# chenc10/distributed_TensorFlow_models

Hardware: AMD Instinct MI355X
Metric: images/sec (whole node) ResNet-50 224×224 bf16 at 1/2/4/8 MI355X (higher is better)
Workload: dtype bf16; 1 GPU; model=resnet_v1_50, global_batch=256, per_gpu_batch=256, image_size=224, parallelism=dp1, device=cuda, grad_allreduce_dtype=fp32, deterministic=True, optimizer=momentum-sgd+wd

## Files before the change

### csrc/kernels/batchnorm.hip

```cpp
#include "common.h"

namespace dtm {

template <int V>
struct Vec;
template <>
struct Vec<8> {
  uint4 u;
  __device__ __forceinline__ void load(const bf16_t* p) { u = *(const uint4*)p; }
  __device__ __forceinline__ void store(bf16_t* p) const { *(uint4*)p = u; }
  __device__ __forceinline__ float get(int e) const {
    uint32_t w = e < 2 ? u.x : e < 4 ? u.y : e < 6 ? u.z : u.w;
    return (e & 1) ? hi_bf(w) : lo_bf(w);
  }
  __device__ __forceinline__ void unpack(float* f) const {
    f[0] = lo_bf(u.x); f[1] = hi_bf(u.x); f[2] = lo_bf(u.y); f[3] = hi_bf(u.y);
    f[4] = lo_bf(u.z); f[5] = hi_bf(u.z); f[6] = lo_bf(u.w); f[7] = hi_bf(u.w);
  }
  __device__ __forceinline__ void pack(const float* f) {
    u = make_uint4(pack2bf(f[0], f[1]), pack2bf(f[2], f[3]), pack2bf(f[4], f[5]), pack2bf(f[6], f[7]));
  }
};
template <>
struct Vec<1> {
// ... 249 lines not shown
}


__global__ __launch_bounds__(256) void bn_stats_fast(const bf16_t* __restrict__ x, float* __restrict__ stats, int M,
                                                     int C, int rpb) {
  __shared__ float red[2][256][8];
  const int cols = C >> 3, t = threadIdx.x, RP = 256 / cols, c0 = (t % cols) * 8, lr0 = t / cols;
  const int r0 = blockIdx.x * rpb, r1 = min(M, r0 + rpb);
  float s[8], q[8];
#pragma unroll
  for (int e = 0; e < 8; ++e) s[e] = q[e] = 0.f;
  for (int r = lr0 < RP ? r0 + lr0 : r1; r < r1; r += RP * FU) {
    uint4 v[FU];
#pragma unroll
    for (int u = 0; u < FU; ++u) {
      int rr = r + u * RP;
      v[u] = rr < r1 ? *(const uint4*)(x + (size_t)rr * C + c0) : make_uint4(0, 0, 0, 0);
    }
#pragma unroll
    for (int u = 0; u < FU; ++u) {
      float f[8]; unpack8(v[u], f);
#pragma unroll
      for (int e = 0; e < 8; ++e) { s[e] += f[e]; q[e] += f[e] * f[e]; }
    }
  }
  col_reduce8(red, s, q, stats + (size_t)blockIdx.x * 2 * C, stats + (size_t)blockIdx.x * 2 * C + C, cols, c0);
}

typedef unsigned int v4u_bn_t __attribute__((ext_vector_type(4)));
template <bool NT>
__device__ __forceinline__ uint4 ld16_bn(const bf16_t* p) {
  if (NT) {
    v4u_bn_t v = __builtin_nontemporal_load((const v4u_bn_t*)p);
    return make_uint4(v.x, v.y, v.z, v.w);
  }
  return *(const uint4*)p;
}

template <bool NT>
__global__ __launch_bounds__(256) void bn_apply_fast(const bf16_t* __restrict__ x, const float* __restrict__ ss,
                                                     const bf16_t* __restrict__ res, const float* __restrict__ rss,
                                                     bf16_t* __restrict__ y, uint8_t* __restrict__ mask, int M, int C,
                                                     int res_mode, int relu, int rpb, int ldy) {
  const int cols = C >> 3, t = threadIdx.x, RP = 256 / cols, c0 = (t % cols) * 8, lr0 = t / cols;
  float sc[8], sh[8], rsc[8], rsh[8];
#pragma unroll
  for (int e = 0; e < 8; ++e) {
    sc[e] = ss[c0 + e]; sh[e] = ss[C + c0 + e];
    rsc[e] = res_mode == 2 ? rss[c0 + e] : 1.f;
    rsh[e] = res_mode == 2 ? rss[C + c0 + e] : 0.f;
  }
  const int r0 = blockIdx.x * rpb, r1 = min(M, r0 + rpb);
  for (int r = lr0 < RP ? r0 + lr0 : r1; r < r1; r += RP * FU) {
    uint4 v[FU], w[FU];
#pragma unroll
    for (int u = 0; u < FU; ++u) {
      int rr = r + u * RP;
      bool ok = rr < r1;
      v[u] = ok ? ld16_bn<NT>(x + (size_t)rr * C + c0) : make_uint4(0, 0, 0, 0);
      if (res_mode) w[u] = ok ? ld16_bn<NT>(res + (size_t)rr * C + c0) : make_uint4(0, 0, 0, 0);
    }
#pragma unroll
    for (int u = 0; u < FU; ++u) {
      int rr = r + u * RP;
      if (rr >= r1) break;
      float f[8]; unpack8(v[u], f);
#pragma unroll
      for (int e = 0; e < 8; ++e) f[e] = fmaf(f[e], sc[e], sh[e]);
      if (res_mode) {
        float g[8]; unpack8(w[u], g);
#pragma unroll
        for (int e = 0; e < 8; ++e) f[e] += fmaf(g[e], rsc[e], rsh[e]);
      }
      if (relu) {
        uint32_t bits = 0;
#pragma unroll
        for (int e = 0; e < 8; ++e) {
          bits |= (f[e] > 0.f ? 1u : 0u) << e;
          f[e] = fmaxf(f[e], 0.f);
        }
        if (mask) mask[((size_t)rr * C + c0) >> 3] = (uint8_t)bits;
      }
      *(uint4*)(y + (size_t)rr * ldy + c0) = pack8(f);
    }
  }
}

__global__ __launch_bounds__(256) void bn_apply_res_strided(const bf16_t* __restrict__ x, const float* __restrict__ ss,
                                                            const bf16_t* __restrict__ res, bf16_t* __restrict__ y,
                                                            uint8_t* __restrict__ mask,
                                                            uint32_t M, int C, int relu, FastDiv fd_cols, FastDiv fd_Wo,
                                                            FastDiv fd_Ho, int Ho, int Wo, int Hi, int Wi, int s) {
  const uint32_t cols = C >> 3, total = M * cols;
  for (uint32_t i = blockIdx.x * 256u + threadIdx.x; i < total; i += gridDim.x * 256u) {
    const uint32_t r = fdiv(i, fd_cols), c0 = (i - r * cols) * 8;
    const uint32_t t = fdiv(r, fd_Wo), w = r - t * Wo;
    const uint32_t n = fdiv(t, fd_Ho), h = t - n * Ho;
    const size_t rr = ((size_t)n * Hi + (size_t)h * s) * Wi + (size_t)w * s;
    float f[8], g[8];
    unpack8(*(const uint4*)(x + (size_t)r * C + c0), f);
    unpack8(*(const uint4*)(res + rr * C + c0), g);
    uint32_t bits = 0;
#pragma unroll
    for (int e = 0; e < 8; ++e) {
      f[e] = fmaf(f[e], ss[c0 + e], ss[C + c0 + e]) + g[e];
      bits |= (f[e] > 0.f ? 1u : 0u) << e;
      if (relu) f[e] = fmaxf(f[e], 0.f);
    }
    if (relu && mask) mask[((size_t)r * C + c0) >> 3] = (uint8_t)bits;
    *(uint4*)(y + (size_t)r * C + c0) = pack8(f);
  }
}

__global__ __launch_bounds__(256) void bn_bwd_reduce_fast(const bf16_t* __restrict__ dy, const bf16_t* __restrict__ x,
                                                          const bf16_t* __restrict__ ym, const float* __restrict__ ss,
                                                          float* __restrict__ sums, int M, int C, int mask_mode, int rpb) {
  __shared__ float red[2][256][8];
  const int cols = C >> 3, t = threadIdx.x, RP = 256 / cols, c0 = (t % cols) * 8, lr0 = t / cols;
  float sc[8], sh[8], mu[8], rs[8];
#pragma unroll
  for (int e = 0; e < 8; ++e) {
    sc[e] = ss[c0 + e]; sh[e] = ss[C + c0 + e]; mu[e] = ss[2 * C + c0 + e]; rs[e] = ss[3 * C + c0 + e];
  }
  const int r0 = blockIdx.x * rpb, r1 = min(M, r0 + rpb);
  float s[8], q[8];
#pragma unroll
  for (int e = 0; e < 8; ++e) s[e] = q[e] = 0.f;
  for (int r = lr0 < RP ? r0 + lr0 : r1; r < r1; r += RP * FU) {
    uint4 a[FU], b[FU], m[FU];
#pragma unroll
    for (int u = 0; u < FU; ++u) {
      int rr = r + u * RP;
      bool ok = rr < r1;
      size_t o = (size_t)rr * C + c0;
      a[u] = ok ? *(const uint4*)(dy + o) : make_uint4(0, 0, 0, 0);
      b[u] = ok ? *(const uint4*)(x + o) : make_uint4(0, 0, 0, 0);
      if (mask_mode == 1) m[u] = ok ? *(const uint4*)(ym + o) : make_uint4(0, 0, 0, 0);
    }
#pragma unroll
    for (int u = 0; u < FU; ++u) {
      float g[8], xv[8];
      unpack8(a[u], g); unpack8(b[u], xv);
      if (mask_mode == 1) {
        float mv[8]; unpack8(m[u], mv);
#pragma unroll
        for (int e = 0; e < 8; ++e) g[e] = mv[e] > 0.f ? g[e] : 0.f;
      } else if (mask_mode == 2) {
#pragma unroll
        for (int e = 0; e < 8; ++e) g[e] = fmaf(xv[e], sc[e], sh[e]) > 0.f ? g[e] : 0.f;
      }
#pragma unroll
      for (int e = 0; e < 8; ++e) { s[e] += g[e]; q[e] += g[e] * (xv[e] - mu[e]) * rs[e]; }
    }
  }
  col_reduce8(red, s, q, sums + (size_t)blockIdx.x * 2 * C, sums + (size_t)blockIdx.x * 2 * C + C, cols, c0);
}

__global__ __launch_bounds__(256) void bn_bwd_apply_fast(const bf16_t* __restrict__ dy, const bf16_t* __restrict__ x,
                                                         const bf16_t* __restrict__ ym, const float* __restrict__ ss,
                                                         const float* __restrict__ sums, bf16_t* __restrict__ dx,
                                                         bf16_t* __restrict__ gout, int M, int C, int mask_mode,
                                                         int training, int rpb) {
  const int cols = C >> 3, t = threadIdx.x, RP = 256 / cols, c0 = (t % cols) * 8, lr0 = t / cols;
  const float invM = 1.f / (float)M;
  float sc[8], sh[8], mu[8], rs[8], A[8], Bq[8];
#pragma unroll
// ... 222 lines not shown
  long blocks = (n8 + 255) / 256;
  if (blocks > 8192) blocks = 8192;
  hipLaunchKernelGGL(bn_stats_bwd_kernel, dim3((unsigned)blocks), dim3(256), 0, (hipStream_t)stream, (const bf16_t*)y,
                     dstats, (const bf16_t*)g, (bf16_t*)dy, n8, C / 8);
  return 0;
}

DTM_API void dtm_bn_stats(const void* x, float* stats, long M, int C, void* stream) {
  if (fast_ok(M, C)) {
    int blocks, rpb; fast_grid(M, C, &blocks, &rpb);
    float* ws = dtm_ws_get_stream((size_t)blocks * 2 * C, (hipStream_t)stream);
    hipLaunchKernelGGL(bn_stats_fast, dim3(blocks), dim3(256), 0, (hipStream_t)stream, (const bf16_t*)x, ws, (int)M, C, rpb);
    dtm_reduce_rows(ws, blocks, 2 * C, 2 * C, stats, (hipStream_t)stream);
    return;
  }
  long rpb = rows_per_block_for(M, C);
  int blocks = (int)((M + rpb - 1) / rpb);
  if (C % 8 == 0)
    hipLaunchKernelGGL(bn_stats_kernel<8>, dim3(blocks), dim3(256), 0, (hipStream_t)stream, (const bf16_t*)x, stats, M, C, rpb);
  else
    hipLaunchKernelGGL(bn_stats_kernel<1>, dim3(blocks), dim3(256), 0, (hipStream_t)stream, (const bf16_t*)x, stats, M, C, rpb);
}

DTM_API int dtm_col_sums(const void* x, float* stats, long M, int C, void* stream) {
  if (!fast_ok(M, C)) return -1;
  int blocks, rpb; fast_grid(M, C, &blocks, &rpb);
  float* ws = dtm_ws_get_stream((size_t)blocks * 2 * C, (hipStream_t)stream);
  if (!ws) return -4;
  hipLaunchKernelGGL(bn_stats_fast, dim3(blocks), dim3(256), 0, (hipStream_t)stream, (const bf16_t*)x, ws, (int)M, C, rpb);
  dtm_reduce_rows_det(ws, blocks, 2 * C, 2 * C, stats, (hipStream_t)stream);
  return 0;
}

DTM_API void dtm_bn_finalize(const float* stats, const float* gamma, const float* beta, float* mov_mean,
                             float* mov_var, float* out, int C, float count, float eps, float decay, int update,
                             int bessel, void* stream) {
  hipLaunchKernelGGL(bn_finalize_kernel, dim3((C + 255) / 256), dim3(256), 0, (hipStream_t)stream, stats, gamma, beta,
                     mov_mean, mov_var, out, C, count, eps, decay, update, bessel);
}

DTM_API void dtm_bn_inference_params(const float* gamma, const float* beta, const float* mov_mean,
                                     const float* mov_var, float* out, int C, float eps, void* stream) {
  hipLaunchKernelGGL(bn_inference_params_kernel, dim3((C + 255) / 256), dim3(256), 0, (hipStream_t)stream, gamma, beta,
                     mov_mean, mov_var, out, C, eps);
}

DTM_API int dtm_bn_apply2(const void* x, const float* ss, const void* res, const float* rss, void* y, void* mask, long M,
                          int C, int res_mode, int relu, void* stream) {
  if (fast_ok(M, C)) {
    int blocks, rpb; fast_grid(M, C, &blocks, &rpb);
    hipLaunchKernelGGL((dtm_ntld_bits() & 1) ? bn_apply_fast<true> : bn_apply_fast<false>, dim3(blocks), dim3(256), 0, (hipStream_t)stream, (const bf16_t*)x, ss,
                       (const bf16_t*)res, rss, (bf16_t*)y, (uint8_t*)mask, (int)M, C, res_mode, relu, rpb, C);
    return 0;
  }
  if (mask) return -7;
  if (C % 8 == 0)
    hipLaunchKernelGGL(bn_apply_kernel<8>, dim3(grid_for(M * C / 8)), dim3(256), 0, (hipStream_t)stream,
                       (const bf16_t*)x, ss, (const bf16_t*)res, rss, (bf16_t*)y, M, C, res_mode, relu);
  else
    hipLaunchKernelGGL(bn_apply_kernel<1>, dim3(grid_for(M * C)), dim3(256), 0, (hipStream_t)stream,
                       (const bf16_t*)x, ss, (const bf16_t*)res, rss, (bf16_t*)y, M, C, res_mode, relu);
  return 0;
}

DTM_API int dtm_bn_apply_ld(const void* x, const float* ss, void* y, void* mask, long M, int C, int relu, int ldy,
                            void* stream) {
  if (!fast_ok(M, C) || ldy < C || ldy % 8 || ((uintptr_t)y & 15) || M * (long)ldy >= (1l << 40)) return -1;
  int blocks, rpb; fast_grid(M, C, &blocks, &rpb);
  hipLaunchKernelGGL((dtm_ntld_bits() & 1) ? bn_apply_fast<true> : bn_apply_fast<false>, dim3(blocks), dim3(256), 0, (hipStream_t)stream, (const bf16_t*)x, ss,
                     (const bf16_t*)nullptr, (const float*)nullptr, (bf16_t*)y, (uint8_t*)mask, (int)M, C, 0, relu, rpb,
                     ldy);
  return 0;
}

DTM_API void dtm_bn_apply(const void* x, const float* ss, const void* res, const float* rss, void* y, long M, int C,
                          int res_mode, int relu, void* stream) {
  dtm_bn_apply2(x, ss, res, rss, y, nullptr, M, C, res_mode, relu, stream);
}

DTM_API int dtm_bn_apply_res_strided(const void* x, const float* ss, const void* res, void* y, void* mask, int N, int Ho,
                                     int Wo, int C, int Hi, int Wi, int s, int relu, void* stream) {
  if (C % 8 || (long)N * Ho * Wo * (C / 8) >= (1l << 31) || (Ho - 1) * s >= Hi || (Wo - 1) * s >= Wi) return -1;
  const uint32_t M = (uint32_t)N * Ho * Wo;
  const long total = (long)M * (C / 8);
  long blocks = (total + 255) / 256;
  if (blocks > 8192) blocks = 8192;
  hipLaunchKernelGGL(bn_apply_res_strided, dim3((int)blocks), dim3(256), 0, (hipStream_t)stream, (const bf16_t*)x, ss,
                     (const bf16_t*)res, (bf16_t*)y, (uint8_t*)mask, M, C, relu, make_fastdiv(C / 8), make_fastdiv(Wo),
                     make_fastdiv(Ho), Ho, Wo, Hi, Wi, s);
  return 0;
}

DTM_API void dtm_bn_bwd_reduce(const void* dy, const void* x, const void* ymask, const float* ss, float* sums, long M,
                               int C, int mask_mode, void* stream) {
  if (fast_ok(M, C)) {
    int blocks, rpb; fast_grid(M, C, &blocks, &rpb);
    float* ws = dtm_ws_get_stream((size_t)blocks * 2 * C, (hipStream_t)stream);
    hipLaunchKernelGGL(bn_bwd_reduce_fast, dim3(blocks), dim3(256), 0, (hipStream_t)stream, (const bf16_t*)dy,
                       (const bf16_t*)x, (const bf16_t*)ymask, ss, ws, (int)M, C, mask_mode, rpb);
    dtm_reduce_rows(ws, blocks, 2 * C, 2 * C, sums, (hipStream_t)stream);
    return;
  }
  long rpb = rows_per_block_for(M, C);
  int blocks = (int)((M + rpb - 1) / rpb);
  if (C % 8 == 0)
    hipLaunchKernelGGL(bn_bwd_reduce_kernel<8>, dim3(blocks), dim3(256), 0, (hipStream_t)stream, (const bf16_t*)dy,
                       (const bf16_t*)x, (const bf16_t*)ymask, ss, sums, M, C, mask_mode, rpb);
  else
    hipLaunchKernelGGL(bn_bwd_reduce_kernel<1>, dim3(blocks), dim3(256), 0, (hipStream_t)stream, (const bf16_t*)dy,
                       (const bf16_t*)x, (const bf16_t*)ymask, ss, sums, M, C, mask_mode, rpb);
}

DTM_API void dtm_bn_bwd_apply(const void* dy, const void* x, const void* ymask, const float* ss, const float* sums,
                              void* dx, void* gout, long M, int C, int mask_mode, int training, void* stream) {
  if (fast_ok(M, C)) {
    int blocks, rpb; fast_grid(M, C, &blocks, &rpb);
    hipLaunchKernelGGL(bn_bwd_apply_fast, dim3(blocks), dim3(256), 0, (hipStream_t)stream, (const bf16_t*)dy,
                       (const bf16_t*)x, (const bf16_t*)ymask, ss, sums, (bf16_t*)dx, (bf16_t*)gout, (int)M, C,
                       mask_mode, training, rpb);
    return;
  }
  if (C % 8 == 0)
    hipLaunchKernelGGL(bn_bwd_apply_kernel<8>, dim3(grid_for(M * C / 8)), dim3(256), 0, (hipStream_t)stream,
                       (const bf16_t*)dy, (const bf16_t*)x, (const bf16_t*)ymask, ss, sums, (bf16_t*)dx, (bf16_t*)gout,
                       M, C, mask_mode, training);
  else
    hipLaunchKernelGGL(bn_bwd_apply_kernel<1>, dim3(grid_for(M * C)), dim3(256), 0, (hipStream_t)stream,
                       (const bf16_t*)dy, (const bf16_t*)x, (const bf16_t*)ymask, ss, sums, (bf16_t*)dx, (bf16_t*)gout,
                       M, C, mask_mode, training);
}

DTM_API void dtm_bn_param_grad(const float* sums, float* dgamma, float* dbeta, int C, void* stream) {
  hipLaunchKernelGGL(bn_param_grad_kernel, dim3((C + 255) / 256), dim3(256), 0, (hipStream_t)stream, sums, dgamma,
                     dbeta, C);
}

static float* g_fin_acc[DTM_WS_SLOTS] = {};
static unsigned* g_fin_counter[DTM_WS_SLOTS] = {};
static int g_fin_k[DTM_WS_SLOTS] = {};

int dtm_bn_stats_finalize(const float* ws, int rows, int K, const float* gamma, const float* beta, float* mov_mean,
                          float* mov_var, float* ss, float count, float eps, float decay, int update, int bessel,
                          hipStream_t st) {
  return dtm_bn_stats_finalize_g(ws, rows, K, gamma, beta, mov_mean, mov_var, ss, count, eps, decay, update, bessel, st,
                                 nullptr);
}
int dtm_bn_stats_finalize_g(const float* ws, int rows, int K, const float* gamma, const float* beta, float* mov_mean,
                            float* mov_var, float* ss, float count, float eps, float decay, int update, int bessel,
                            hipStream_t st, const FinGroup* fg) {
  if (!dtm_device_ok()) return -9;
  const int k = dtm_ws_slot(st);
  if (K > g_fin_k[k]) {
    if (dtm_stream_capturing(st)) {
      dtm_ws_set_error(-10);
      return -4;
    }
    unsigned* cnt = nullptr;
    float* acc = nullptr;
    if (hipMalloc(&cnt, 64) != hipSuccess) return -4;
    if (hipMalloc(&acc, (size_t)2 * K * sizeof(float)) != hipSuccess) return -4;
    hipMemsetAsync(acc, 0, (size_t)2 * K * sizeof(float), st);
    hipMemsetAsync(cnt, 0, 64, st);
    if (g_fin_acc[k]) dtm_ws_note_retired();
    g_fin_acc[k] = acc;
    g_fin_counter[k] = cnt;
    g_fin_k[k] = K;
// ... 30 lines not shown
```

### csrc/kernels/conv_igemm.hip

```cpp
#include "common.h"
#include <cstdio>

namespace dtm {


struct ConvNTArgs {
  const bf16_t* x;
  const bf16_t* w;
  bf16_t* y;
  float* stats;
  const float* bias;
  const float* in_scale;
  const float* in_shift;
  uint32_t x_bytes, w_bytes;
  int N, Hin, Win, C, K, R, S, P, Q;
  int stride, pad_h, pad_w;
  int Hv, Wv;
  int M;
  int Kg;
  int relu;
  FastDiv fd_PQ, fd_Q;
  const bf16_t* add_src;
  int add_stride;
  int add_H, add_W;
// ... 2178 lines not shown
  typedef __attribute__((address_space(3))) short4v lds_s4;
  typedef __attribute__((address_space(3))) char lds_c;
  short8 P[2][4], Wa[2][2], Wb[2][2];
  auto frag = [&](const char* half, int ks, int m) -> short8 {
    lds_c* lb = (lds_c*)half;
    const int kb = ks * 32 + 8 * lg;
    const short4v lo = __builtin_amdgcn_ds_read_tr16_b64_v4i16((lds_s4*)(lb + tr_off<128>(kb + tq, m)));
    const short4v hi = __builtin_amdgcn_ds_read_tr16_b64_v4i16((lds_s4*)(lb + tr_off<128>(kb + 4 + tq, m)));
    return (short8){lo[0], lo[1], lo[2], lo[3], hi[0], hi[1], hi[2], hi[3]};
  };
  auto rd_p = [&](const char* s, int mi) {
#pragma unroll
    for (int ks = 0; ks < 2; ++ks)
#pragma unroll
      for (int jj = 0; jj < 4; ++jj) P[ks][jj] = frag(s + mi * HALF, ks, grp * 64 + jj * 16 + 4 * tp);
  };
  auto rd_w = [&](const char* s, int ni) {
#pragma unroll
    for (int ks = 0; ks < 2; ++ks)
#pragma unroll
      for (int ii = 0; ii < 2; ++ii) {
        const short8 v = frag(s + (2 + ni) * HALF, ks, wq * 32 + ii * 16 + 4 * tp);
        if (ni == 0) Wa[ks][ii] = v;
        else Wb[ks][ii] = v;
      }
  };
  auto mma = [&](int ni, int mi) {
#pragma unroll
    for (int ks = 0; ks < 2; ++ks)
#pragma unroll
      for (int ii = 0; ii < 2; ++ii)
#pragma unroll
        for (int jj = 0; jj < 4; ++jj)
          acc[ni][ii][mi][jj] = __builtin_amdgcn_mfma_f32_16x16x32_bf16(P[ks][jj], ni == 0 ? Wa[ks][ii] : Wb[ks][ii],
                                                                        acc[ni][ii][mi][jj], 0, 0, 0);
  };
  pp_mainloop(smem, BUF, nk, grp, issue, rd_p, rd_w, mma);

  float* slab = a.dw + (size_t)bz * a.K * a.Kg;
#pragma unroll
  for (int ni = 0; ni < 2; ++ni)
#pragma unroll
    for (int ii = 0; ii < 2; ++ii) {
      const int col = n0 + ni * 128 + wq * 32 + ii * 16 + li;
#pragma unroll
      for (int mi = 0; mi < 2; ++mi)
#pragma unroll
        for (int jj = 0; jj < 4; ++jj) {
          const int ko = m0 + mi * 128 + grp * 64 + jj * 16 + lg * 4;
          if (col < a.Kg) {
#pragma unroll
            for (int r = 0; r < 4; ++r)
              if (ko + r < a.K) slab[(size_t)(ko + r) * a.Kg + col] = acc[ni][ii][mi][jj][r];
          }
        }
    }
}

struct FlipDesc {
  const bf16_t* w;
  bf16_t* wt;
  int K, R, S, C;
  int st, ph, pw, pad_;
};

__host__ __device__ __forceinline__ void dec_dim(int R, int st, int pad, int a, int& r0, int& T, int& off) {
  r0 = ((a + pad) % st + st) % st;
  T = r0 < R ? (R - r0 + st - 1) / st : 0;
  off = (a + pad - r0) / st;
}
__host__ __device__ __forceinline__ size_t dec_block(int R, int S, int C, int K, int st, int ph, int pw, int a, int b) {
  size_t off = 0;
  for (int a2 = 0; a2 < st; ++a2)
    for (int b2 = 0; b2 < st; ++b2) {
      if (a2 == a && b2 == b) return off;
      int r0, Tr, o1, s0, Tu, o2;
      dec_dim(R, st, ph, a2, r0, Tr, o1);
      dec_dim(S, st, pw, b2, s0, Tu, o2);
      off += (size_t)C * K * Tr * Tu;
    }
  return off;
}
constexpr int FLIP_T = 64;
__device__ __forceinline__ void flip_tile(const FlipDesc& f, int tile, uint16_t (*lds)[FLIP_T + 2]) {
  const int kt = (f.K + FLIP_T - 1) / FLIP_T, ct = (f.C + FLIP_T - 1) / FLIP_T;
  const int rs = tile / (kt * ct), rem = tile % (kt * ct);
  const int k0 = (rem / ct) * FLIP_T, c0 = (rem % ct) * FLIP_T;
  const int r = rs / f.S, s = rs % f.S;
  const int rs2 = (f.R - 1 - r) * f.S + (f.S - 1 - s);
  const uint16_t* w = (const uint16_t*)f.w;
  uint16_t* wt = (uint16_t*)f.wt;
  const size_t RS = (size_t)f.R * f.S;
  size_t dRS = RS, drs = rs2;
  if (f.st > 1) {
    const int a = ((r - f.ph) % f.st + f.st) % f.st, b = ((s - f.pw) % f.st + f.st) % f.st;
    int r0, Tr, o1, s0, Tu, o2;
    dec_dim(f.R, f.st, f.ph, a, r0, Tr, o1);
    dec_dim(f.S, f.st, f.pw, b, s0, Tu, o2);
    const int tq = Tr - 1 - (r - r0) / f.st, uq = Tu - 1 - (s - s0) / f.st;
    wt += dec_block(f.R, f.S, f.C, f.K, f.st, f.ph, f.pw, a, b);
    dRS = (size_t)Tr * Tu;
    drs = (size_t)tq * Tu + uq;
  }
#pragma unroll 4
  for (int i = threadIdx.x; i < FLIP_T * FLIP_T; i += 256) {
    const int kk = i / FLIP_T, cc = i % FLIP_T;
    const int k = k0 + kk, c = c0 + cc;
    if (k < f.K && c < f.C) lds[kk][cc] = w[((size_t)k * RS + rs) * f.C + c];
  }
  __syncthreads();
#pragma unroll 4
  for (int i = threadIdx.x; i < FLIP_T * FLIP_T; i += 256) {
    const int cc = i / FLIP_T, kk = i % FLIP_T;
    const int k = k0 + kk, c = c0 + cc;
    if (k < f.K && c < f.C) wt[((size_t)c * dRS + drs) * f.K + k] = lds[kk][cc];
  }
  __syncthreads();
}

__device__ __forceinline__ int flip_tiles(const FlipDesc& f) {
  return ((f.K + FLIP_T - 1) / FLIP_T) * ((f.C + FLIP_T - 1) / FLIP_T) * f.R * f.S;
}

__global__ __launch_bounds__(256) void weight_flip_batched_kernel(const FlipDesc* __restrict__ descs) {
  __shared__ uint16_t lds[FLIP_T][FLIP_T + 2];
  const FlipDesc f = descs[blockIdx.y];
  const int n = flip_tiles(f);
  for (int t = blockIdx.x; t < n; t += gridDim.x) flip_tile(f, t, lds);
}

__global__ __launch_bounds__(256) void weight_flip_tiled_kernel(FlipDesc f) {
  __shared__ uint16_t lds[FLIP_T][FLIP_T + 2];
  const int n = flip_tiles(f);
  for (int t = blockIdx.x; t < n; t += gridDim.x) flip_tile(f, t, lds);
}

}

using namespace dtm;

struct ConvDesc {
  int N, H, W, C, K, R, S, P, Q, stride, pad_h, pad_w;
  int pix_bytes;
  int dec;
};

static const bf16_t* zero_chunk() {
  static void* z = nullptr;
  if (!z) {
    if (hipMalloc(&z, 4096) != hipSuccess) return nullptr;
    hipMemset(z, 0, 4096);
    hipDeviceSynchronize();
  }
  return (const bf16_t*)z;
}
const void* dtm_zero_chunk() { return zero_chunk(); }

template <int PT, int CT, int NWP, int NS, int UD, bool SPL = false, int NTH = 512>
static void launch_w8(const ConvNTArgs& a, hipStream_t st) {
  dim3 grid((a.K + CT - 1) / CT, (a.M + PT - 1) / PT, a.ngrp > 1 ? a.ngrp : 1);
  hipLaunchKernelGGL((conv_nt_w8_kernel<PT, CT, NWP, NS, UD, SPL, NTH>), grid, dim3(NTH), 0, st, a);
}

template <int UD, bool SPL = false>
static void launch_pp(const ConvNTArgs& a, hipStream_t st) {
  dim3 grid((a.K + 255) / 256, (a.M + 255) / 256, a.ngrp > 1 ? a.ngrp : 1);
  hipLaunchKernelGGL((conv_nt_pp_kernel<UD, SPL>), grid, dim3(512), 0, st, a);
}

template <int PT, int CT, int NS, int UD, int NWP = 2, bool SPL = false>
static void launch_pipe(const ConvNTArgs& a, hipStream_t st) {
  dim3 grid((a.K + CT - 1) / CT, (a.M + PT - 1) / PT, a.ngrp > 1 ? a.ngrp : 1);
  if (SPL) hipLaunchKernelGGL((conv_nt_pipe_kernel<PT, CT, NS, UD, false, NWP, true>), grid, dim3(256), 0, st, a);
  else if (a.in_scale) hipLaunchKernelGGL((conv_nt_pipe_kernel<PT, CT, NS, UD, true, NWP>), grid, dim3(256), 0, st, a);
  else hipLaunchKernelGGL((conv_nt_pipe_kernel<PT, CT, NS, UD, false, NWP>), grid, dim3(256), 0, st, a);
}

static int device_cus() { return dtm_compute_cus(); }

static bf16_t* dump_chunk() {
  static void* z = nullptr;
  if (!z && hipMalloc(&z, 4096) != hipSuccess) return nullptr;
  return (bf16_t*)z;
}

template <int PT, int CT, int NKT, bool PRO, bool STEM = false, int NBUF = 2, bool SIDE = true>
static int stream_workers_k(const ConvNTArgs& a) {
  static int occ = 0;
  if (!occ) {
    if (hipOccupancyMaxActiveBlocksPerMultiprocessor(&occ, conv1x1_stream_kernel<PT, CT, NKT, PRO, STEM, NBUF, SIDE>,
                                                     256, 0) !=
            hipSuccess || occ <= 0)
      occ = 1;
  }
  const int ctiles = (a.K + CT - 1) / CT;
  const int ntiles = (a.M + PT - 1) / PT;
  int workers = (occ * device_cus() + ctiles - 1) / ctiles;
  if (workers > ntiles) workers = ntiles;
  if (workers < 1) workers = 1;
  return workers;
}

template <int PT, int CT, int NKT, bool PRO, bool STEM = false, int NBUF = 2, bool SIDE = true>
static void launch_stream_k(const ConvNTArgs& a, hipStream_t st) {
  const int ctiles = (a.K + CT - 1) / CT;
  const int ntiles = (a.M + PT - 1) / PT;
  hipLaunchKernelGGL((conv1x1_stream_kernel<PT, CT, NKT, PRO, STEM, NBUF, SIDE>),
                     dim3(ctiles, stream_workers_k<PT, CT, NKT, PRO, STEM, NBUF, SIDE>(a)), dim3(256), 0, st, a, ntiles);
}

static bool stem_stream_ok(const ConvNTArgs& a) {
  return a.pix_bytes == 8 && a.C == 32 && a.S == 1 && a.pad_h == 0 && a.pad_w == 0 && a.Kg == a.R * 32 &&
         a.Kg <= 256 && a.K % 64 == 0 && !a.in_scale && !a.bias && !a.relu && a.ostr == 1;
}

// ... 716 lines not shown
```

### csrc/kernels/elementwise.hip

```cpp
#include "common.h"

namespace dtm {

__device__ __forceinline__ uint32_t hash_u32(uint64_t seed, uint64_t i) {
  uint64_t z = seed + 0x9E3779B97F4A7C15ull * (i + 1);
  z = (z ^ (z >> 30)) * 0xBF58476D1CE4E5B9ull;
  z = (z ^ (z >> 27)) * 0x94D049BB133111EBull;
  z ^= z >> 31;
  return (uint32_t)(z >> 32);
}

__device__ __forceinline__ uint64_t mix_seed(uint64_t seed, uint64_t off) {
  if (off == 0) return seed;
  uint64_t z = off * 0x9E3779B97F4A7C15ull;
  z = (z ^ (z >> 30)) * 0xBF58476D1CE4E5B9ull;
  z = (z ^ (z >> 27)) * 0x94D049BB133111EBull;
  return seed ^ z ^ (z >> 31);
}

template <bool BF16>
__global__ __launch_bounds__(256) void dropout_kernel(const void* __restrict__ xv, void* __restrict__ yv, long n,
                                                      uint32_t thresh, float inv_keep, uint64_t seed0,
                                                      const unsigned long long* __restrict__ seed_off) {
  const long base = ((long)blockIdx.x * 256 + threadIdx.x) * 8;
  if (base >= n) return;
  const uint64_t seed = seed_off ? mix_seed(seed0, *seed_off) : seed0;
  float v[8];
  if (BF16) {
    const bf16_t* x = (const bf16_t*)xv;
    if (base + 8 <= n) {
      uint4 u = *(const uint4*)(x + base);
      uint32_t w[4] = {u.x, u.y, u.z, u.w};
#pragma unroll
      for (int j = 0; j < 4; ++j) { v[2 * j] = lo_bf(w[j]); v[2 * j + 1] = hi_bf(w[j]); }
    } else {
      for (int j = 0; j < 8; ++j) v[j] = base + j < n ? bf2f(x[base + j]) : 0.f;
    }
  } else {
    const float* x = (const float*)xv;
    if (base + 8 <= n) {
      float4 a = *(const float4*)(x + base), b = *(const float4*)(x + base + 4);
      v[0] = a.x; v[1] = a.y; v[2] = a.z; v[3] = a.w; v[4] = b.x; v[5] = b.y; v[6] = b.z; v[7] = b.w;
    } else {
      for (int j = 0; j < 8; ++j) v[j] = base + j < n ? x[base + j] : 0.f;
    }
  }
#pragma unroll
  for (int j = 0; j < 8; ++j) v[j] = hash_u32(seed, (uint64_t)(base + j)) < thresh ? v[j] * inv_keep : 0.f;
  if (BF16) {
    bf16_t* y = (bf16_t*)yv;
    if (base + 8 <= n) {
      uint4 u;
      u.x = pack2bf(v[0], v[1]); u.y = pack2bf(v[2], v[3]); u.z = pack2bf(v[4], v[5]); u.w = pack2bf(v[6], v[7]);
      *(uint4*)(y + base) = u;
    } else {
      for (int j = 0; j < 8; ++j) if (base + j < n) y[base + j] = f2bf(v[j]);
    }
  } else {
    float* y = (float*)yv;
    if (base + 8 <= n) {
      *(float4*)(y + base) = make_float4(v[0], v[1], v[2], v[3]);
      *(float4*)(y + base + 4) = make_float4(v[4], v[5], v[6], v[7]);
    } else {
      for (int j = 0; j < 8; ++j) if (base + j < n) y[base + j] = v[j];
    }
  }
}

template <bool BF16>
__global__ __launch_bounds__(256) void in_top_k_kernel(const void* __restrict__ logits, const int* __restrict__ labels,
                                                       uint8_t* __restrict__ out, int B, int K, int k) {
  const int row = blockIdx.x * 4 + (threadIdx.x >> 6), lane = threadIdx.x & 63;
  if (row >= B) return;
  const int t = labels[row];
  auto ld = [&](long i) -> float {
    return BF16 ? bf2f(((const bf16_t*)logits)[i]) : ((const float*)logits)[i];
  };
  const long off = (long)row * K;
  const bool valid = t >= 0 && t < K;
  const float xt = valid ? ld(off + t) : 0.f;
  int cnt = 0;
  for (int c = lane; c < K; c += 64) cnt += ld(off + c) > xt ? 1 : 0;
#pragma unroll
  for (int o = 32; o > 0; o >>= 1) cnt += __shfl_xor(cnt, o, 64);
  if (lane == 0) out[row] = (valid && isfinite(xt) && cnt < k) ? 1 : 0;
}

template <bool F32>
__global__ __launch_bounds__(256) void stem_pack_kernel(const void* __restrict__ x, bf16_t* __restrict__ xp, int N,
                                                        int H, int W, int C, int Hp, int Wp, int pad) {
  const long npair = (long)N * Hp * (Wp / 2);
  for (long t = blockIdx.x * 256L + threadIdx.x; t < npair; t += (long)gridDim.x * 256) {
    const int w0 = (int)(t % (Wp / 2)) * 2;
    const long nh = t / (Wp / 2);
    const int h = (int)(nh % Hp), n = (int)(nh / Hp);
    const int ih = h - pad;
    uint32_t o[4] = {0u, 0u, 0u, 0u};
#pragma unroll
    for (int k = 0; k < 2; ++k) {
      const int iw = w0 + k - pad;
      if (ih >= 0 && ih < H && iw >= 0 && iw < W) {
        const long base = (((long)n * H + ih) * W + iw) * C;
        float v[4] = {0.f, 0.f, 0.f, 0.f};
        for (int c = 0; c < C; ++c)
          v[c] = F32 ? ((const float*)x)[base + c] : __uint_as_float((uint32_t)((const uint16_t*)x)[base + c] << 16);
        o[2 * k] = pack2bf(v[0], v[1]);
        o[2 * k + 1] = pack2bf(v[2], v[3]);
      }
    }
    *(uint4*)(xp + (nh * Wp + w0) * 4) = make_uint4(o[0], o[1], o[2], o[3]);
  }
}

}

using namespace dtm;

DTM_API int dtm_stem_pack(const void* x, int dtype, void* xp, int N, int H, int W, int C, int Hp, int Wp, int pad,
                          hipStream_t st) {
  if (C < 1 || C > 4 || (Wp & 1) || ((uintptr_t)xp & 15)) return -1;
  const long npair = (long)N * Hp * (Wp / 2);
  long blocks = (npair + 255) / 256;
  if (blocks > 65536) blocks = 65536;
  if (dtype == 0)
    stem_pack_kernel<true><<<(unsigned)blocks, 256, 0, st>>>(x, (bf16_t*)xp, N, H, W, C, Hp, Wp, pad);
  else
    stem_pack_kernel<false><<<(unsigned)blocks, 256, 0, st>>>(x, (bf16_t*)xp, N, H, W, C, Hp, Wp, pad);
  return hipGetLastError() == hipSuccess ? 0 : 2;
}

DTM_API int dtm_dropout(const void* x, void* y, long n, int dtype, float keep_prob, unsigned long long seed,
                        const unsigned long long* seed_off, hipStream_t st) {
  if (n <= 0) return 0;
  if (!(keep_prob > 0.f && keep_prob <= 1.f)) return 1;
  const double t = (double)keep_prob * 4294967296.0;
  const uint32_t thresh = t >= 4294967295.0 ? 0xFFFFFFFFu : (uint32_t)t;
  const long threads = (n + 7) / 8;
  const unsigned grid = (unsigned)((threads + 255) / 256);
  if (dtype == 1)
    dropout_kernel<true><<<grid, 256, 0, st>>>(x, y, n, thresh, 1.f / keep_prob, seed, seed_off);
  else
    dropout_kernel<false><<<grid, 256, 0, st>>>(x, y, n, thresh, 1.f / keep_prob, seed, seed_off);
  return hipGetLastError() == hipSuccess ? 0 : 2;
}

DTM_API int dtm_in_top_k(const void* logits, const int* labels, uint8_t* out, int B, int K, int k, int dtype,
                         hipStream_t st) {
  if (B <= 0) return 0;
  const unsigned grid = (unsigned)((B + 3) / 4);
  if (dtype == 1)
    in_top_k_kernel<true><<<grid, 256, 0, st>>>(logits, labels, out, B, K, k);
  else
    in_top_k_kernel<false><<<grid, 256, 0, st>>>(logits, labels, out, B, K, k);
  return hipGetLastError() == hipSuccess ? 0 : 2;
}
```

### csrc/kernels/fused_bn.hip

```cpp
#include <cstring>

#include "common.h"

namespace dtm {

constexpr int FU2 = 4;

__device__ __forceinline__ void up8(uint4 u, float* f) {
  f[0] = lo_bf(u.x); f[1] = hi_bf(u.x); f[2] = lo_bf(u.y); f[3] = hi_bf(u.y);
  f[4] = lo_bf(u.z); f[5] = hi_bf(u.z); f[6] = lo_bf(u.w); f[7] = hi_bf(u.w);
}
__device__ __forceinline__ uint4 pk8(const float* f) {
  return make_uint4(pack2bf(f[0], f[1]), pack2bf(f[2], f[3]), pack2bf(f[4], f[5]), pack2bf(f[6], f[7]));
}


typedef unsigned int v4u_t __attribute__((ext_vector_type(4)));
template <bool NT>
__device__ __forceinline__ uint4 ld16(const bf16_t* p) {
  if (NT) {
    v4u_t v = __builtin_nontemporal_load((const v4u_t*)p);
    return make_uint4(v.x, v.y, v.z, v.w);
  }
  return *(const uint4*)p;
// ... 123 lines not shown
#pragma unroll
    for (int u = 0; u < FU2; ++u) {
      int rr = row + u * RP;
      if (rr >= r1) break;
      float d[8], xv[8];
      up8(vd[u], d); up8(vx[u], xv);
#pragma unroll
      for (int e = 0; e < 8; ++e) d[e] += a[e] + b[e] * xv[e];
      *(uint4*)(out + (size_t)rr * C + c0) = pk8(d);
    }
  }
}

template <int U, bool NT, bool NTS = NT>
__global__ __launch_bounds__(256) void stats_combine_fin_kernel(const bf16_t* __restrict__ dy, const bf16_t* __restrict__ x,
                                                                const float* __restrict__ dss, const float* __restrict__ ss,
                                                                const float* __restrict__ gamma, float count,
                                                                float* __restrict__ dgamma, float* __restrict__ dbeta,
                                                                bf16_t* __restrict__ out, int M, int C, int prescale,
                                                                int rpb, int ldo) {
  __shared__ float s_ab[2][2048];
  const int cols = C >> 3, t = threadIdx.x, RP = 256 / cols, c0 = (t % cols) * 8, lr0 = t / cols;
  for (int c = t; c < C; c += 256) {
    float ds, dq, dg, db;
    fin_bwd_channel(dss, ss, gamma, C, c, count, &ds, &dq, &dg, &db);
    s_ab[0][c] = ds;
    s_ab[1][c] = 2.f * dq;
    if (blockIdx.x == 0) {
      if (dgamma) dgamma[c] += dg;
      if (dbeta) dbeta[c] += db;
    }
  }
  __syncthreads();
  float a[8], b[8], sc[8];
#pragma unroll
  for (int e = 0; e < 8; ++e) {
    a[e] = s_ab[0][c0 + e];
    b[e] = s_ab[1][c0 + e];
    sc[e] = prescale ? ss[c0 + e] : 1.f;
  }
  const int r0 = blockIdx.x * rpb, r1 = min(M, r0 + rpb);
  for (int row = lr0 < RP ? r0 + lr0 : r1; row < r1; row += RP * U) {
    uint4 vd[U], vx[U];
#pragma unroll
    for (int u = 0; u < U; ++u) {
      int rr = row + u * RP;
      bool ok = rr < r1;
      size_t o = (size_t)rr * C + c0;
      vd[u] = ok ? ld16<NT>(dy + o) : make_uint4(0, 0, 0, 0);
      vx[u] = ok ? ld16<NT>(x + o) : make_uint4(0, 0, 0, 0);
    }
#pragma unroll
    for (int u = 0; u < U; ++u) {
      int rr = row + u * RP;
      if (rr >= r1) break;
      float d[8], xv[8];
      up8(vd[u], d); up8(vx[u], xv);
#pragma unroll
      for (int e = 0; e < 8; ++e) d[e] = fmaf(d[e], sc[e], a[e] + b[e] * xv[e]);
      st16<NTS>(out + (size_t)rr * ldo + c0, pk8(d));
    }
  }
}

__global__ void bn_finalize_bwd_kernel(const float* __restrict__ dss, const float* __restrict__ ss,
                                       const float* __restrict__ gamma, float* __restrict__ dstats,
                                       float* __restrict__ dgamma, float* __restrict__ dbeta, int C, float count) {
  int c = blockIdx.x * blockDim.x + threadIdx.x;
  if (c >= C) return;
  const float scale = ss[c], mean = ss[2 * C + c], rstd = ss[3 * C + c];
  const float g = gamma ? gamma[c] : 1.f;
  const float dsc = dss[c], dsh = dss[C + c];
  const float dscale_tot = dsc - dsh * mean;
  const float dmean = dss[2 * C + c] - dsh * scale;
  const float drstd = dss[3 * C + c] + dscale_tot * g;
  if (dgamma) dgamma[c] += dscale_tot * rstd;
  if (dbeta) dbeta[c] += dsh;
  const float dvar = drstd * (-0.5f) * rstd * rstd * rstd;
  dstats[c] = dmean / count - dvar * 2.f * mean / count;
  dstats[C + c] = dvar / count;
}

static int g_sc_var = 5, g_sc_cap = 4096;
static int g_ntld = 3;

constexpr int CAT_MAXP = 8;
struct CatPart {
  const bf16_t* raw;
  const float* ss;
  uint8_t* mask;
  bf16_t* dx;
  int C, off, flags;
};
struct CatArgs {
  CatPart p[CAT_MAXP];
  int np, Ct, M, rpb;
};
__device__ __forceinline__ int cat_part(const CatArgs& a, int gc) {
  int k = 0;
#pragma unroll
  for (int i = 1; i < CAT_MAXP; ++i)
    if (i < a.np && gc >= a.p[i].off) k = i;
  return k;
}

__global__ __launch_bounds__(256) void cat_bn_apply_kernel(CatArgs a, bf16_t* __restrict__ out) {
  const int cols = a.Ct >> 3, t = threadIdx.x, RP = 256 / cols, gc = (t % cols) * 8, lr0 = t / cols;
  if (lr0 >= RP) return;
  const int k = cat_part(a, gc);
  const CatPart& P = a.p[k];
  const int cl = gc - P.off;
  const bool relu = P.flags & 1, plain = P.flags & 2;
  float sc[8], sh[8];
#pragma unroll
  for (int e = 0; e < 8; ++e) {
    sc[e] = plain ? 1.f : P.ss[cl + e];
    sh[e] = plain ? 0.f : P.ss[P.C + cl + e];
  }
  const int r0 = blockIdx.x * a.rpb, r1 = min(a.M, r0 + a.rpb);
  for (int row = r0 + lr0; row < r1; row += RP * FU2) {
    uint4 v[FU2];
#pragma unroll
    for (int u = 0; u < FU2; ++u) {
      const int rr = row + u * RP;
      v[u] = rr < r1 ? ld16<true>(P.raw + (size_t)rr * P.C + cl) : make_uint4(0, 0, 0, 0);
    }
#pragma unroll
    for (int u = 0; u < FU2; ++u) {
      const int rr = row + u * RP;
      if (rr >= r1) break;
      if (plain) {
        *(uint4*)(out + (size_t)rr * a.Ct + gc) = v[u];
        continue;
      }
      float f[8];
      up8(v[u], f);
      uint32_t bits = 0u;
#pragma unroll
      for (int e = 0; e < 8; ++e) {
        f[e] = fmaf(f[e], sc[e], sh[e]);
        if (relu) f[e] = fmaxf(f[e], 0.f);
        bits |= (f[e] > 0.f ? 1u : 0u) << e;
      }
      *(uint4*)(out + (size_t)rr * a.Ct + gc) = pk8(f);
      if (P.mask) P.mask[((size_t)rr * P.C + cl) >> 3] = (uint8_t)bits;
    }
  }
}

template <int NT>
__global__ __launch_bounds__(NT) void cat_bn_apply_bwd_kernel(CatArgs a, const bf16_t* __restrict__ dout,
                                                              float* __restrict__ ws) {
  __shared__ float red[2][NT][8];
  const int cols = a.Ct >> 3, t = threadIdx.x, RP = NT / cols, gc = (t % cols) * 8, lr0 = t / cols;
  const int k = cat_part(a, gc);
  const CatPart& P = a.p[k];
  const int cl = gc - P.off;
  const bool ux = P.flags & 1, plain = P.flags & 2;
  float sc[8];
#pragma unroll
  for (int e = 0; e < 8; ++e) sc[e] = plain ? 1.f : P.ss[cl + e];
  float a1[8], a0[8];
#pragma unroll
  for (int e = 0; e < 8; ++e) a1[e] = a0[e] = 0.f;
  const int r0 = blockIdx.x * a.rpb, r1 = min(a.M, r0 + a.rpb);
  for (int row = (lr0 < RP && !plain) ? r0 + lr0 : r1; row < r1; row += RP * FU2) {
    uint4 vd[FU2], vx[FU2];
// ... 297 lines not shown
```

Baseline: 15370 images/sec.

## Vectorize strided residual BN, weight flip, and stem pack kernels; enable NT loads

Adds a row-blocked bn_apply_res_strided_fast kernel that loads several rows at once, with optional nontemporal loads, replacing per-element fastdiv indexing. Weight flip gains a 16-byte vectorized path that transposes through swizzled LDS. Stem pack is rewritten to stage input rows in LDS with vectorized loads. The default g_ntld bits now include bit 4, so the new strided kernel uses nontemporal loads. These target memory-bound small kernels, and each is only a minor share of the ResNet-50 step.

```diff
diff --git a/csrc/kernels/batchnorm.hip b/csrc/kernels/batchnorm.hip
--- a/csrc/kernels/batchnorm.hip
+++ b/csrc/kernels/batchnorm.hip
@@ -355,6 +355,48 @@
         if (mask) mask[((size_t)rr * C + c0) >> 3] = (uint8_t)bits;
       }
       *(uint4*)(y + (size_t)rr * ldy + c0) = pack8(f);
+    }
+  }
+}
+
+template <bool NT>
+__global__ __launch_bounds__(256) void bn_apply_res_strided_fast(
+    const bf16_t* __restrict__ x, const float* __restrict__ ss, const bf16_t* __restrict__ res, bf16_t* __restrict__ y,
+    uint8_t* __restrict__ mask, int M, int C, int relu, int rpb, FastDiv fd_Wo, FastDiv fd_Ho, int Ho, int Wo, int Hi,
+    int Wi, int s) {
+  const int cols = C >> 3, t = threadIdx.x, RP = 256 / cols, c0 = (t % cols) * 8, lr0 = t / cols;
+  float sc[8], sh[8];
+#pragma unroll
+  for (int e = 0; e < 8; ++e) { sc[e] = ss[c0 + e]; sh[e] = ss[C + c0 + e]; }
+  const int r0 = blockIdx.x * rpb, r1 = min(M, r0 + rpb);
+  for (int r = lr0 < RP ? r0 + lr0 : r1; r < r1; r += RP * FU) {
+    uint4 v[FU], w[FU];
+#pragma unroll
+    for (int u = 0; u < FU; ++u) {
+      const int rr = r + u * RP;
+      const bool ok = rr < r1;
+      const uint32_t ro = ok ? (uint32_t)rr : 0u;
+      const uint32_t q = fdiv(ro, fd_Wo), wo = ro - q * Wo;
+      const uint32_t n = fdiv(q, fd_Ho), ho = q - n * Ho;
+      const size_t sr = ((size_t)n * Hi + (size_t)ho * s) * Wi + (size_t)wo * s;
+      v[u] = ok ? ld16_bn<NT>(x + (size_t)rr * C + c0) : make_uint4(0, 0, 0, 0);
+      w[u] = ok ? *(const uint4*)(res + sr * C + c0) : make_uint4(0, 0, 0, 0);
+    }
+#pragma unroll
+    for (int u = 0; u < FU; ++u) {
+      const int rr = r + u * RP;
+      if (rr >= r1) break;
+      float f[8], g[8];
+      unpack8(v[u], f); unpack8(w[u], g);
+      uint32_t bits = 0;
+#pragma unroll
+      for (int e = 0; e < 8; ++e) {
+        f[e] = fmaf(f[e], sc[e], sh[e]) + g[e];
+        bits |= (f[e] > 0.f ? 1u : 0u) << e;
+        if (relu) f[e] = fmaxf(f[e], 0.f);
+      }
+      if (relu && mask) mask[((size_t)rr * C + c0) >> 3] = (uint8_t)bits;
+      *(uint4*)(y + (size_t)rr * C + c0) = pack8(f);
     }
   }
 }
@@ -743,6 +785,14 @@
                                      int Wo, int C, int Hi, int Wi, int s, int relu, void* stream) {
   if (C % 8 || (long)N * Ho * Wo * (C / 8) >= (1l << 31) || (Ho - 1) * s >= Hi || (Wo - 1) * s >= Wi) return -1;
   const uint32_t M = (uint32_t)N * Ho * Wo;
+  if (fast_ok(M, C)) {
+    int blocks, rpb; fast_grid(M, C, &blocks, &rpb);
+    hipLaunchKernelGGL((dtm_ntld_bits() & 4) ? bn_apply_res_strided_fast<true> : bn_apply_res_strided_fast<false>,
+                       dim3(blocks), dim3(256), 0, (hipStream_t)stream, (const bf16_t*)x, ss, (const bf16_t*)res,
+                       (bf16_t*)y, (uint8_t*)mask, (int)M, C, relu, rpb, make_fastdiv(Wo), make_fastdiv(Ho), Ho, Wo, Hi,
+                       Wi, s);
+    return 0;
+  }
   const long total = (long)M * (C / 8);
   long blocks = (total + 255) / 256;
   if (blocks > 8192) blocks = 8192;
diff --git a/csrc/kernels/conv_igemm.hip b/csrc/kernels/conv_igemm.hip
--- a/csrc/kernels/conv_igemm.hip
+++ b/csrc/kernels/conv_igemm.hip
@@ -2284,7 +2284,10 @@
   return off;
 }
 constexpr int FLIP_T = 64;
-__device__ __forceinline__ void flip_tile(const FlipDesc& f, int tile, uint16_t (*lds)[FLIP_T + 2]) {
+constexpr int FLIP_LDW = 36;
+constexpr int FLIP_LDS_DWORDS = FLIP_T * FLIP_LDW;
+__device__ __forceinline__ void flip_tile(const FlipDesc& f, int tile, uint32_t* smem) {
+  uint16_t (*lds)[FLIP_T + 2] = (uint16_t (*)[FLIP_T + 2])smem;
   const int kt = (f.K + FLIP_T - 1) / FLIP_T, ct = (f.C + FLIP_T - 1) / FLIP_T;
   const int rs = tile / (kt * ct), rem = tile % (kt * ct);
   const int k0 = (rem / ct) * FLIP_T, c0 = (rem % ct) * FLIP_T;
@@ -2304,6 +2307,35 @@
     dRS = (size_t)Tr * Tu;
     drs = (size_t)tq * Tu + uq;
   }
+  if (!((f.K | f.C) & 7) && !(((uintptr_t)f.w | (uintptr_t)f.wt) & 15)) {
+    {
+      const int kp = threadIdx.x >> 3, ch = threadIdx.x & 7;
+      const int k = k0 + 2 * kp, c = c0 + ch * 8;
+      uint4 a = make_uint4(0, 0, 0, 0), b = a;
+      if (c < f.C) {
+        if (k < f.K) a = *(const uint4*)(w + ((size_t)k * RS + rs) * f.C + c);
+        if (k + 1 < f.K) b = *(const uint4*)(w + ((size_t)(k + 1) * RS + rs) * f.C + c);
+      }
+      const uint32_t av[4] = {a.x, a.y, a.z, a.w}, bv[4] = {b.x, b.y, b.z, b.w};
+      uint32_t* dst = smem + (ch * 8) * FLIP_LDW + (kp ^ (ch << 2));
+#pragma unroll
+      for (int q = 0; q < 4; ++q) {
+        dst[(2 * q) * FLIP_LDW] = (av[q] & 0xffffu) | (bv[q] << 16);
+        dst[(2 * q + 1) * FLIP_LDW] = (av[q] >> 16) | (bv[q] & 0xffff0000u);
+      }
+    }
+    __syncthreads();
+#pragma unroll
+    for (int j = threadIdx.x; j < FLIP_T * 8; j += 256) {
+      const int cc = j >> 3, kch = j & 7;
+      const int c = c0 + cc, k = k0 + kch * 8;
+      if (c < f.C && k < f.K)
+        *(uint4*)(wt + ((size_t)c * dRS + drs) * f.K + k) =
+            *(const uint4*)(smem + cc * FLIP_LDW + ((kch ^ (cc >> 3)) << 2));
+    }
+    __syncthreads();
+    return;
+  }
 #pragma unroll 4
   for (int i = threadIdx.x; i < FLIP_T * FLIP_T; i += 256) {
     const int kk = i / FLIP_T, cc = i % FLIP_T;
@@ -2325,14 +2357,14 @@
 }
 
 __global__ __launch_bounds__(256) void weight_flip_batched_kernel(const FlipDesc* __restrict__ descs) {
-  __shared__ uint16_t lds[FLIP_T][FLIP_T + 2];
+  __shared__ __attribute__((aligned(16))) uint32_t lds[FLIP_LDS_DWORDS];
   const FlipDesc f = descs[blockIdx.y];
   const int n = flip_tiles(f);
   for (int t = blockIdx.x; t < n; t += gridDim.x) flip_tile(f, t, lds);
 }
 
 __global__ __launch_bounds__(256) void weight_flip_tiled_kernel(FlipDesc f) {
-  __shared__ uint16_t lds[FLIP_T][FLIP_T + 2];
+  __shared__ __attribute__((aligned(16))) uint32_t lds[FLIP_LDS_DWORDS];
   const int n = flip_tiles(f);
   for (int t = blockIdx.x; t < n; t += gridDim.x) flip_tile(f, t, lds);
 }
diff --git a/csrc/kernels/elementwise.hip b/csrc/kernels/elementwise.hip
--- a/csrc/kernels/elementwise.hip
+++ b/csrc/kernels/elementwise.hip
@@ -86,30 +86,69 @@
   if (lane == 0) out[row] = (valid && isfinite(xt) && cnt < k) ? 1 : 0;
 }
 
+constexpr int STEM_LDS = 2048;
 template <bool F32>
-__global__ __launch_bounds__(256) void stem_pack_kernel(const void* __restrict__ x, bf16_t* __restrict__ xp, int N,
-                                                        int H, int W, int C, int Hp, int Wp, int pad) {
-  const long npair = (long)N * Hp * (Wp / 2);
-  for (long t = blockIdx.x * 256L + threadIdx.x; t < npair; t += (long)gridDim.x * 256) {
-    const int w0 = (int)(t % (Wp / 2)) * 2;
-    const long nh = t / (Wp / 2);
-    const int h = (int)(nh % Hp), n = (int)(nh / Hp);
-    const int ih = h - pad;
-    uint32_t o[4] = {0u, 0u, 0u, 0u};
+__global__ __launch_bounds__(256) void stem_pack_kernel(const void* __restrict__ x, bf16_t* __restrict__ xp, long rows,
+                                                        int H, int W, int C, int Hp, int Wp, int pad, int TP, int RB,
+                                                        int LDR, int vec) {
+  __shared__ __attribute__((aligned(16))) uint16_t sm[STEM_LDS];
+  const long row0 = (long)blockIdx.x * RB;
+  const int w_s = blockIdx.y * 2 * TP;
+  const int i_s = max(0, w_s - pad), i_e = min(W, w_s + 2 * TP - pad);
+  const int ne = max(0, i_e - i_s) * C;
+  const int t = threadIdx.x;
+  if (vec) {
+    const int cpr = F32 ? ne >> 2 : ne >> 3;
+    for (int q = t; q < RB * cpr; q += 256) {
+      const int rb = q / cpr, cq = q - rb * cpr;
+      const long row = row0 + rb;
+      const int ih = (int)(row % Hp) - pad;
+      if (row >= rows || ih < 0 || ih >= H) continue;
+      const size_t src = ((size_t)(row / Hp) * H + ih) * W * C;
+      if (F32) {
+        const float4 v = ((const float4*)((const float*)x + src))[cq];
+        *(uint2*)(sm + rb * LDR + cq * 4) = make_uint2(pack2bf(v.x, v.y), pack2bf(v.z, v.w));
+      } else {
+        const uint4 v = ((const uint4*)((const uint16_t*)x + src))[cq];
+        *(uint4*)(sm + rb * LDR + cq * 8) =
+            make_uint4(pack2bf(lo_bf(v.x), hi_bf(v.x)), pack2bf(lo_bf(v.y), hi_bf(v.y)),
+                       pack2bf(lo_bf(v.z), hi_bf(v.z)), pack2bf(lo_bf(v.w), hi_bf(v.w)));
+      }
+    }
+  } else {
+    for (int rb = 0; rb < RB; ++rb) {
+      const long row = row0 + rb;
+      const int ih = (int)(row % Hp) - pad;
+      if (row >= rows || ih < 0 || ih >= H) continue;
+      const size_t src = (((size_t)(row / Hp) * H + ih) * W + i_s) * C;
+      for (int e = t; e < ne; e += 256)
+        sm[rb * LDR + e] = f2bf(F32 ? ((const float*)x)[src + e]
+                                    : __uint_as_float((uint32_t)((const uint16_t*)x)[src + e] << 16));
+    }
+  }
+  __syncthreads();
+  if (t >= RB * TP) return;
+  const int rb = t / TP, w0 = w_s + 2 * (t - rb * TP);
+  const long row = row0 + rb;
+  if (row >= rows || w0 >= Wp) return;
+  const int ih = (int)(row % Hp) - pad;
+  uint32_t o[4] = {0u, 0u, 0u, 0u};
+  if (ih >= 0 && ih < H) {
 #pragma unroll
     for (int k = 0; k < 2; ++k) {
       const int iw = w0 + k - pad;
-      if (ih >= 0 && ih < H && iw >= 0 && iw < W) {
-        const long base = (((long)n * H + ih) * W + iw) * C;
-        float v[4] = {0.f, 0.f, 0.f, 0.f};
-        for (int c = 0; c < C; ++c)
-          v[c] = F32 ? ((const float*)x)[base + c] : __uint_as_float((uint32_t)((const uint16_t*)x)[base + c] << 16);
-        o[2 * k] = pack2bf(v[0], v[1]);
-        o[2 * k + 1] = pack2bf(v[2], v[3]);
+      if (iw >= 0 && iw < W) {
+        const uint16_t* px = sm + rb * LDR + (iw - i_s) * C;
+        uint32_t v[4] = {0u, 0u, 0u, 0u};
+#pragma unroll
+        for (int c = 0; c < 4; ++c)
+          if (c < C) v[c] = px[c];
+        o[2 * k] = v[0] | (v[1] << 16);
+        o[2 * k + 1] = v[2] | (v[3] << 16);
       }
     }
-    *(uint4*)(xp + (nh * Wp + w0) * 4) = make_uint4(o[0], o[1], o[2], o[3]);
-  }
+  }
+  *(uint4*)(xp + ((size_t)row * Wp + w0) * 4) = make_uint4(o[0], o[1], o[2], o[3]);
 }
 
 }
@@ -118,14 +157,21 @@
 
 DTM_API int dtm_stem_pack(const void* x, int dtype, void* xp, int N, int H, int W, int C, int Hp, int Wp, int pad,
                           hipStream_t st) {
-  if (C < 1 || C > 4 || (Wp & 1) || ((uintptr_t)xp & 15)) return -1;
-  const long npair = (long)N * Hp * (Wp / 2);
-  long blocks = (npair + 255) / 256;
-  if (blocks > 65536) blocks = 65536;
+  if (C < 1 || C > 4 || (Wp & 1) || ((uintptr_t)xp & 15) || pad < 0 || W < 1 || pad + W > Wp) return -1;
+  const long rows = (long)N * Hp;
+  if (rows <= 0 || Wp <= 0) return 0;
+  const int pairs = Wp / 2, TP = pairs < 256 ? pairs : 256;
+  const int LDR = (2 * TP * C + 7) & ~7;
+  int RB = 256 / TP;
+  if (RB > STEM_LDS / LDR) RB = STEM_LDS / LDR;
+  const long bx = (rows + RB - 1) / RB;
+  if (bx >= (1l << 31)) return -1;
+  const int vec = pairs <= 256 && !((uintptr_t)x & 15) && (W * C) % (dtype == 0 ? 4 : 8) == 0;
+  const dim3 grid((unsigned)bx, (unsigned)((pairs + TP - 1) / TP));
   if (dtype == 0)
-    stem_pack_kernel<true><<<(unsigned)blocks, 256, 0, st>>>(x, (bf16_t*)xp, N, H, W, C, Hp, Wp, pad);
+    stem_pack_kernel<true><<<grid, 256, 0, st>>>(x, (bf16_t*)xp, rows, H, W, C, Hp, Wp, pad, TP, RB, LDR, vec);
   else
-    stem_pack_kernel<false><<<(unsigned)blocks, 256, 0, st>>>(x, (bf16_t*)xp, N, H, W, C, Hp, Wp, pad);
+    stem_pack_kernel<false><<<grid, 256, 0, st>>>(x, (bf16_t*)xp, rows, H, W, C, Hp, Wp, pad, TP, RB, LDR, vec);
   return hipGetLastError() == hipSuccess ? 0 : 2;
 }
 
diff --git a/csrc/kernels/fused_bn.hip b/csrc/kernels/fused_bn.hip
--- a/csrc/kernels/fused_bn.hip
+++ b/csrc/kernels/fused_bn.hip
@@ -229,7 +229,7 @@
 }
 
 static int g_sc_var = 5, g_sc_cap = 4096;
-static int g_ntld = 3;
+static int g_ntld = 7;
 
 constexpr int CAT_MAXP = 8;
 struct CatPart {
```

New measurement: 15470 images/sec (median of 6 runs). About the same (+0.6%).
